# sandyresearch/chipmunk

Measured on AMD Instinct MI355X. Metric: DiT denoise steps/sec at fixed sparsity, higher is better.
Workload: dtype bf16

## Files before the change

### chipmunk_amd/csrc/attn64.hip

```cpp
#include "common.h"
#include "attn64_regs.h"
#include "attn_params.h"
#include "attn64_util.h"
#include <type_traits>

namespace {

constexpr int HD = 128;
constexpr int KT = 64;
constexpr int WROWS = 64, WGROWS = 256;
constexpr int TB = KT * HD * 2;
constexpr int NSL = 4;
constexpr int VRING = NSL * TB;
constexpr int LDS_BYTES = 2 * NSL * TB;
constexpr int PSTAGE = 64 * 128;
constexpr int LDS_BYTES_CSUM = LDS_BYTES + 4 * PSTAGE;
constexpr int CS_EXCH_BYTES = 2 * 4 * 64 * 4;
constexpr float SCALE_LOG2E = 0.08838834764f * 1.44269504089f;
constexpr float MAX_LAG = 4.0f;
#ifndef A64_ABL
#define A64_ABL 0
#endif
#ifndef A64_EB
#define A64_EB 20
#endif
#ifndef A64_EA
#define A64_EA 35
#endif
#ifndef A64_CSUM_VALU
#define A64_CSUM_VALU 1
#endif
#ifndef A64_VSPREAD
#define A64_VSPREAD 0
#endif
#ifndef A64_DMA_POS
#define A64_DMA_POS 2
#endif

constexpr int a64_ecum(int k) {
    return k <= 0 ? 0 : k <= 20 ? (k * A64_EB) / 20 : k <= 52 ? A64_EB + ((k - 20) * A64_EA) / 32
                                                              : (A64_EB + A64_EA + (k - 52) < 64 ? A64_EB + A64_EA + (k - 52) : 64);
}
constexpr int a64_cstep(int j) {
    int k = 0;
    while (a64_ecum(k) < 2 * j + 2) ++k;
    return k;
}
constexpr int a64_rk(int u) { return u == 0 ? 36 : u == 1 ? 38 : u == 2 ? 68 : 70; }
constexpr int a64_mk(int u) { return u == 0 ? 46 : u == 1 ? 48 : u == 2 ? 78 : 80; }

#ifdef ATTN64_PROF
__device__ unsigned long long g_a64_prof[4 * 8];
#define P64_DECL unsigned long long pt_ = 0, pacc_[7] = {0, 0, 0, 0, 0, 0, 0}; const bool prof_on_ = blockIdx.x == (gridDim.x / 2)
#define P64_START() do { if (prof_on_) pt_ = __builtin_amdgcn_s_memtime(); } while (0)
#define P64_MARK(i) do { if (prof_on_) { const unsigned long long n_ = __builtin_amdgcn_s_memtime(); pacc_[i] += n_ - pt_; pt_ = n_; } } while (0)
#define P64_END(w, n) do { if (prof_on_ && lane == 0) { for (int i_ = 0; i_ < 7; ++i_) g_a64_prof[(w) * 8 + i_] = pacc_[i_]; g_a64_prof[(w) * 8 + 7] = (n); } } while (0)
#else
#define P64_DECL
#define P64_START()
#define P64_MARK(i)
#define P64_END(w, n)
#endif

template <int KB, int QB, int KS>
__device__ __forceinline__ void mfma_qk(f32x16 &s) {
    constexpr int ka = 192 + (KB * 8 + KS) * 4, qa = 128 + (QB * 8 + KS) * 4;
    if constexpr (A64_ABL & 64) {
        constexpr int oa = (KB * 2 + QB) * 16;
        asm volatile("v_mfma_f32_32x32x16_bf16 a[%c0:%c1], a[%c2:%c3], a[%c4:%c5], a[%c0:%c1]" ::"i"(oa), "i"(oa + 15), "i"(ka), "i"(ka + 3), "i"(qa), "i"(qa + 3));
        return;
    }
    if constexpr (KS == 0)
        asm volatile("v_mfma_f32_32x32x16_bf16 %0, a[%c1:%c2], a[%c3:%c4], 0" : "=v"(s) : "i"(ka), "i"(ka + 3), "i"(qa), "i"(qa + 3));
    else
        asm volatile("v_mfma_f32_32x32x16_bf16 %0, a[%c1:%c2], a[%c3:%c4], %0" : "+v"(s) : "i"(ka), "i"(ka + 3), "i"(qa), "i"(qa + 3));
}
template <int QB, int DB>
__device__ __forceinline__ void mfma_pv(const u32x4 &vf, const u32x4 &pf) {
    constexpr int oa = (QB * 4 + DB) * 16;
    asm volatile("v_mfma_f32_32x32x16_bf16 a[%c2:%c3], %0, %1, a[%c2:%c3]" ::"v"(vf), "v"(pf), "i"(oa), "i"(oa + 15));
}
template <int KB, int KS, int SLOT>
__device__ __forceinline__ void lds_k(uint32_t addr) {
    constexpr int ka = 192 + (KB * 8 + KS) * 4;
    asm volatile("ds_read_b128 a[%c1:%c2], %0 offset:%c3" ::"v"(addr), "i"(ka), "i"(ka + 3), "i"(SLOT * TB + KB * 8192) : "memory");
}
__device__ __forceinline__ void cs_pair16x2(float &a, float &b, float &c, float &d) {
    asm volatile("v_permlane16_swap_b32 %0, %1\n\tv_permlane16_swap_b32 %2, %3\n\tv_add_f32 %0, %0, %1\n\tv_add_f32 %2, %2, %3"
                 : "+v"(a), "+v"(b), "+v"(c), "+v"(d));
}
__device__ __forceinline__ void cs_pair8(float &a, const float &b) {
    asm volatile("v_add_f32_dpp %0, %0, %0 row_mirror row_mask:0xf bank_mask:0x3\n\t"
                 "v_add_f32_dpp %0, %1, %1 row_mirror row_mask:0xf bank_mask:0xc" : "+v"(a) : "v"(b));
}
__device__ __forceinline__ void cs_pair4(float &a, const float &b) {
    asm volatile("v_add_f32_dpp %0, %0, %0 row_half_mirror row_mask:0xf bank_mask:0x5\n\t"
                 "v_add_f32_dpp %0, %1, %1 row_half_mirror row_mask:0xf bank_mask:0xa" : "+v"(a) : "v"(b));
}
template <int CTRL>
__device__ __forceinline__ float cs_pair_quad(float a, float b, bool hi) {
    const float keep = hi ? b : a, give = hi ? a : b;
    return keep + __uint_as_float((uint32_t)__builtin_amdgcn_update_dpp(0, (int)__float_as_uint(give), CTRL, 0xf, 0xf, true));
}
__global__ __launch_bounds__(256) void knorm_max_kernel(const uint16_t *k, const int64_t ks0, const int64_t ks1, const int64_t ks2, int H, int Nk,
                                                        float *out) {
    const int bh = blockIdx.y, b = bh / H, h = bh - b * H;
    const uint16_t *kb = k + b * ks0 + h * ks1;
    const int grp = threadIdx.x >> 4, li = threadIdx.x & 15;
    float best = 0.f;
#pragma unroll 4
    for (int row = blockIdx.x * 16 + grp; row < Nk; row += gridDim.x * 16) {
        const u32x4 v = *(const u32x4 *)(kb + (int64_t)row * ks2 + li * 8);
        float ss = 0.f;
#pragma unroll
        for (int e = 0; e < 4; ++e) {
            const float lo = __uint_as_float(v[e] << 16), hi = __uint_as_float(v[e] & 0xffff0000u);
            ss = __builtin_fmaf(lo, lo, ss);
            ss = __builtin_fmaf(hi, hi, ss);
        }
        best = fmaxf(best, row16_sum(ss));
    }
    __shared__ float red[256];
    red[threadIdx.x] = best;
    __syncthreads();
    for (int st = 128; st > 0; st >>= 1) {
        if ((int)threadIdx.x < st) red[threadIdx.x] = fmaxf(red[threadIdx.x], red[threadIdx.x + st]);
        __syncthreads();
    }
    if (threadIdx.x == 0) atomicMax((unsigned int *)(out + bh), __float_as_uint(__builtin_sqrtf(red[0])));
}

template <int MODE>
__global__ __launch_bounds__(256) __attribute__((amdgpu_waves_per_eu(1, 1))) void attn64_kernel(const AttnParams p) {
    constexpr bool GATHER = MODE == 1 || MODE == 2, INPLACE = MODE == 2;
    constexpr bool CSUM = MODE == 3;
    extern __shared__ __attribute__((aligned(16))) unsigned char smem[];
    const int tid = threadIdx.x, lane = tid & 63;
    const int w = __builtin_amdgcn_readfirstlane(tid >> 6);
    const int l31 = lane & 31, hf = lane >> 5, l15 = lane & 15, lg = lane >> 4;
// ... 43 lines not shown
#pragma unroll
                for (int j = 0; j < 16; ++j) {
                    int pos = base + j;
                    pos = pos < irow.width ? pos : irow.width - 1;
                    dst[j] = idx[pos];
                }
            }
#pragma unroll
            for (int j = 0; j < 16; ++j) dst[j] = max(0, min(dst[j], p.Nk - 1));
        };
        auto all_k = [&](const int (&src)[16], int slot) {
#pragma unroll
            for (int pc = 0; pc < 16; ++pc) blds16(krsrc, __umul24((uint32_t)src[pc], kstride_b) + kswz[pc & 3], 0, smem + slot * TB + pc * 1024);
        };
        auto all_v = [&](const int (&src)[16], int slot) {
#pragma unroll
            for (int pc = 0; pc < 16; ++pc) blds16(vrsrc, __umul24((uint32_t)src[pc], vstride_b) + vswz, 0, smem + VRING + slot * TB + pc * 1024);
        };
        load_idx(0, ir[0]), load_idx(1, ir[1]), load_idx(2, ir[2]), load_idx(3, ir[3]);
        all_k(ir[0], 0);
        all_k(ir[1], 1), all_v(ir[0], 3);
        all_k(ir[2], 2), all_v(ir[0], 0);
        all_k(ir[3], 3), all_v(ir[1], 1);
        load_idx(4, ir[0]);
        asm volatile("s_waitcnt vmcnt(0)" ::: "memory");
        __syncthreads();
        auto loader_tile = [&](auto slc, int t) __attribute__((always_inline)) {
            constexpr int SL = decltype(slc)::value;
            asm volatile("s_waitcnt vmcnt(63)" ::: "memory");
            __builtin_amdgcn_s_barrier();
            load_idx(t + 5, ir[(SL + 1) & 3]);
            all_k(ir[SL], SL);
            all_v(ir[(SL + 2) & 3], (SL + 2) & 3);
        };
        for (int tb = 0;; tb += 4) {
            loader_tile(ic<0>{}, tb);
            if (tb >= T4) break;
            loader_tile(ic<1>{}, tb + 1);
            loader_tile(ic<2>{}, tb + 2);
            loader_tile(ic<3>{}, tb + 3);
        }
        asm volatile("s_waitcnt vmcnt(0)" ::: "memory");
        if (nsp > 1) {
            __syncthreads();
            __syncthreads();
            if (*(volatile int *)(smem) != nsp - 1) return;
            __syncthreads();
        }
        return;
    }

    asm volatile(A64_ZERO_O ::: A64_CLOBBER_ALL);
    float qss[2] = {0.f, 0.f};
    {
        const uint16_t *qp = p.q + b * p.qs[0] + h * p.qs[1];
        static_for<0, 16>([&](auto f) {
            constexpr int F = decltype(f)::value, qb = F >> 3, ks = F & 7;
            const int qrow = row0 + qb * 32 + l31;
            u32x4 val = {0u, 0u, 0u, 0u};
            if (qrow < p.Nq) val = *(const u32x4 *)(qp + (int64_t)qrow * p.qs[2] + ks * 16 + hf * 8);
            acc_write4<128 + F * 4>(val);
#pragma unroll
            for (int e = 0; e < 4; ++e) {
                const float lo = __uint_as_float(val[e] << 16), hi = __uint_as_float(val[e] & 0xffff0000u);
                qss[qb] = __builtin_fmaf(lo, lo, qss[qb]);
                qss[qb] = __builtin_fmaf(hi, hi, qss[qb]);
            }
        });
    }

    const uint32_t lds0 = (uint32_t)(uintptr_t)(__attribute__((address_space(3))) unsigned char *)smem;
    uint32_t kad[8];
#pragma unroll
    for (int ks = 0; ks < 8; ++ks) kad[ks] = lds0 + l31 * 256 + (((2 * ks + hf) ^ l15) << 4);
    uint32_t vad[4];
#pragma unroll
    for (int db = 0; db < 4; ++db)
        vad[db] = lds0 + VRING + (4 * hf + (l15 >> 2)) * 256 + (((db * 4 + 2 * (lg & 1) + ((l15 & 3) >> 1)) ^ ((l15 >> 2) << 2)) << 4) +
                  (l15 & 1) * 8;
    uint32_t kofs[4];
#pragma unroll
    for (int i = 0; i < 4; ++i) kofs[i] = (uint32_t)(w * 16 + 4 * i + lg) * kstride_b + ((uint32_t)(l15 ^ (4 * i + lg)) << 4);
    const uint32_t vofs = (uint32_t)(w * 16 + lg) * vstride_b + ((uint32_t)(l15 ^ (lg << 2)) << 4);

    const int last_base = p.Nk - KT;
    auto tile_base = [&](int T) { return T * KT < last_base ? T * KT : last_base; };
    auto issue_k1 = [&](uint32_t soff, uint32_t ldsw, int slot, int i) {
        blds16(krsrc, kofs[i], soff, smem + ldsw + slot * TB + i * 1024);
    };
    auto issue_v1 = [&](uint32_t soff, uint32_t ldsw, int slot, int i) {
        blds16(vrsrc, vofs, soff + (uint32_t)(4 * i) * vstride_b, smem + ldsw + VRING + slot * TB + i * 1024);
    };
    auto issue_k = [&](int T, int slot) {
        const uint32_t soff = (uint32_t)tile_base(T) * kstride_b;
#pragma unroll
        for (int i = 0; i < 4; ++i) issue_k1(soff, w * 4096, slot, i);
    };
    auto issue_v = [&](int T, int slot) {
        const uint32_t soff = (uint32_t)tile_base(T) * vstride_b;
#pragma unroll
        for (int i = 0; i < 4; ++i) issue_v1(soff, w * 4096, slot, i);
    };

    if constexpr (!GATHER) {
        issue_k(0, 0);
        issue_k(1, 1), issue_v(0, 3);
        issue_k(2, 2), issue_v(0, 0);
        issue_k(3, 3), issue_v(1, 1);
        asm volatile("s_waitcnt vmcnt(24)" ::: "memory");
    }
    __syncthreads();
    static_for<0, 16>([&](auto i) {
        constexpr int I = decltype(i)::value;
        lds_k<(I >> 3), (I & 7), 0>(kad[I & 7]);
    });
    asm volatile("s_waitcnt lgkmcnt(0)" ::: "memory");

    f32x16 s[4];
    float px[64];
    uint32_t pw[2][4][4] = {};
    float m[2] = {-INFINITY, -INFINITY}, nmsc[2] = {0.f, 0.f};
    float mlag[2] = {-INFINITY, -INFINITY};
    float lacc[2][2] = {{0.f, 0.f}, {0.f, 0.f}};
    float alpha[2] = {1.f, 1.f};
    float wq[2] = {0.f, 0.f}, lpq[2] = {-1.0e30f, -1.0e30f}, c4[2] = {0.f, 0.f}, c5 = 0.f;
    uint32_t csoff = 0, ex_w = 0, ex_r = 0;
    int cs_extra = 0;
    float cs_own = 0.f;
    __amdgpu_buffer_rsrc_t prsrc = krsrc;
    uint32_t pst_w = 0, pst_r = 0, csoff_mx = 0;
    u32x2 csf[8] = {};
    f32x4 csacc[2] = {{0.f, 0.f, 0.f, 0.f}, {0.f, 0.f, 0.f, 0.f}};
    float csout = 0.f;
    u32x4 cs_ones = {0x3f803f80u, 0x3f803f80u, 0x3f803f80u, 0x3f803f80u};
    if constexpr (CSUM) {
        static_assert(A64_CSUM_VALU, "the matrix-pipe column-sum probe (A64_CSUM_VALU=0) fills all 160 KiB of LDS with its P stage: no room for the exchange area of the in-workgroup combine; build round 5's tree for it");
        pin(cs_ones);
        const uint32_t pst = lds0 + LDS_BYTES + (uint32_t)w * PSTAGE;
        pst_w = pst + l31 * 128 + ((uint32_t)(hf ^ (l31 & 7)) << 4);
        const int prow = lg * 4 + (l15 >> 2);
        pst_r = pst + prow * 128 + ((uint32_t)(((l15 & 3) >> 1) ^ (prow & 7)) << 4) + (l15 & 1) * 8;
        csoff_mx = 2u * (uint32_t)(16 * lg + 8 * ((l15 >> 2) & 1) + 4 * (l15 >> 3) + (l15 & 3));
#pragma unroll
        for (int qb = 0; qb < 2; ++qb) {
            const int qrow = row0 + qb * 32 + l31;
            const float pl = qrow < p.Nq ? p.p_in[(int64_t)bh * p.Nq + qrow] : 0.f;
            lpq[qb] = pl > 0.f ? __builtin_amdgcn_logf(pl) : -1.0e30f;
        }
        const int rr = ((lane >> 4) & 1) | (((lane >> 3) & 1) << 1) | (((lane >> 2) & 1) << 2);
        csoff = 2u * (uint32_t)(32 * (lane & 1) + (rr & 3) + 8 * (2 * ((lane >> 1) & 1) + (rr >> 2)) + 4 * hf);
        const int nA = 3 - (4 * g) % 3;
        const int lead = w < nA ? 0 : nA, members = w < nA ? nA : 4 - nA;
        cs_extra = w == lead ? members : 0;
        ex_w = lds0 + LDS_BYTES + (uint32_t)w * 256u + (uint32_t)lane * 4u;
        ex_r = lds0 + LDS_BYTES + (uint32_t)(lead + 1) * 256u + (uint32_t)lane * 4u;
        prsrc = make_rsrc(p.cs_part + ((int64_t)bh * (p.G * 2) + (g * 2 + (w < nA ? 0 : 1))) * p.cs_pstride);
    }
#pragma unroll
    for (int e = 0; e < 64; ++e) px[e] = e < 20 ? 0.f : -INFINITY;

    auto vfrag_read = [&](auto dbc, auto offc) __attribute__((always_inline)) {
        constexpr int DB = decltype(dbc)::value, OFF = decltype(offc)::value;
        u32x2 lo, hi;
        asm volatile("ds_read_b64_tr_b16 %0, %2 offset:%c3\n\tds_read_b64_tr_b16 %1, %2 offset:%c4"
                     : "=&v"(lo), "=&v"(hi) : "v"(vad[DB]), "i"(OFF), "i"(OFF + 2048) : "memory");
        return (u32x4){lo[0], lo[1], hi[0], hi[1]};
    };

    static_assert(64 - A64_EB - A64_EA >= 0 && 64 - A64_EB - A64_EA <= 9, "the last steps must finish before gap 12 of the next PV phase");
    auto ecum = [](int k) constexpr { return a64_ecum(k); };
    auto finish_step = [&](auto kk, auto uwc) __attribute__((always_inline)) {
        constexpr int K = decltype(kk)::value;
        constexpr bool UW = decltype(uwc)::value != 0;
        if constexpr (!(A64_ABL & 1)) {
            static_for<ecum(K), ecum(K + 1)>([&](auto ii) {
                constexpr int I = decltype(ii)::value;
                if constexpr (A64_ABL & 32) px[I] = px[I] * 0.5f;
                else px[I] = __builtin_amdgcn_exp2f(px[I]);
                pin(px[I]);
            });
            static_for<ecum(K - 1), ecum(K)>([&](auto ii) {
                constexpr int I = decltype(ii)::value;
                lacc[(I >> 3) & 1][I & 1] += px[I];
                pin(lacc[(I >> 3) & 1][I & 1]);
            });
            static_for<(ecum(K - 1) >> 1), (ecum(K) >> 1)>([&](auto jj) {
                constexpr int J = decltype(jj)::value, I = 2 * J;
                pw[(I >> 3) & 1][I >> 4][(I & 7) >> 1] = pack_bf16x2(px[I], px[I + 1]);
                pin(pw[(I >> 3) & 1][I >> 4][(I & 7) >> 1]);
            });
            if constexpr (CSUM && UW && !A64_CSUM_VALU) {
                static_assert(a64_cstep(8 * 1 + 7) + 1 < a64_rk(0) && a64_cstep(8 * 3 + 7) + 1 < a64_rk(2), "a unit is read after its second fragment is stored");
                static_for<0, 4>([&](auto uu) {
                    constexpr int U = decltype(uu)::value, S = (U & 1) * 4;
                    if constexpr (K == a64_mk(U) || K == a64_mk(U) + 1) {
                        constexpr int H2 = K - a64_mk(U);
                        if constexpr (H2 == 0 && (U & 1) == 0)
                            asm volatile("s_waitcnt lgkmcnt(0)" : "+v"(csf[0]), "+v"(csf[1]), "+v"(csf[2]), "+v"(csf[3]), "+v"(csf[4]), "+v"(csf[5]), "+v"(csf[6]), "+v"(csf[7]) :: "memory");
                        const u32x4 fr = {csf[S + 2 * H2][0], csf[S + 2 * H2][1], csf[S + 2 * H2 + 1][0], csf[S + 2 * H2 + 1][1]};
                        if constexpr (H2 == 0) asm volatile("v_mfma_f32_16x16x32_bf16 %0, %1, %2, 0" : "=&v"(csacc[U & 1]) : "v"(cs_ones), "v"(fr));
                        else asm volatile("v_mfma_f32_16x16x32_bf16 %0, %1, %2, %0" : "+v"(csacc[U & 1]) : "v"(cs_ones), "v"(fr));
                    }
                    if constexpr (K == a64_mk(U) + 3) {
                        if constexpr (U == 0) csout = csacc[0][0];
                        else csout = lg == U ? csacc[U & 1][0] : csout;
                        pin(csout);
                    }
                    if constexpr (K == a64_rk(U) || K == a64_rk(U) + 1) {
                        constexpr int H2 = K - a64_rk(U);
                        uint32_t ad = pst_r;
                        if constexpr (U != 0) ad ^= (uint32_t)(U << 5);
                        asm volatile("ds_read_b64_tr_b16 %0, %2 offset:%c3\n\tds_read_b64_tr_b16 %1, %2 offset:%c4"
                                     : "=&v"(csf[S + 2 * H2]), "=&v"(csf[S + 2 * H2 + 1]) : "v"(ad), "i"(H2 * 4096), "i"(H2 * 4096 + 2048) : "memory");
                    }
                });
                static_for<0, 8>([&](auto ii) {
                    constexpr int U = decltype(ii)::value >> 1, QW = decltype(ii)::value & 1;
                    if constexpr (K == a64_cstep(8 * U + 4 * QW + 3) + 1) {
                        uint32_t ad = pst_w;
                        if constexpr (U != 0) ad ^= (uint32_t)(U << 5);
                        const u32x4 pf = {pw[QW][U][0], pw[QW][U][1], pw[QW][U][2], pw[QW][U][3]};
                        asm volatile("ds_write_b128 %0, %1 offset:%c2" ::"v"(ad), "v"(pf), "i"(QW * 4096) : "memory");
                    }
                });
            } else if constexpr (CSUM) {
                static_for<ecum(K - 3), ecum(K - 2)>([&](auto ii) {
                    constexpr int I = decltype(ii)::value;
                    if constexpr (UW) {
                        if constexpr (((I >> 3) & 1) == 1) { px[I] += px[I - 8]; pin(px[I]); }
                    } else {
                        if constexpr (((I >> 3) & 1) == 0) px[I] *= wq[0];
                        else px[I] = __builtin_fmaf(px[I], wq[1], px[I - 8]);
                        pin(px[I]);
                    }
                });
                static_for<ecum(K - 4), ecum(K - 3)>([&](auto ii) {
                    constexpr int I = decltype(ii)::value;
                    if constexpr ((I & 11) == 11) cs_pair16x2(px[I - 3], px[I - 2], px[I - 1], px[I]);
                });
                static_for<ecum(K - 5), ecum(K - 4)>([&](auto ii) {
                    constexpr int I = decltype(ii)::value;
                    if constexpr ((I & 11) == 11) cs_pair8(px[I - 3], px[I - 1]);
                });
                static_for<ecum(K - 6), ecum(K - 5)>([&](auto ii) {
                    constexpr int I = decltype(ii)::value;
                    if constexpr ((I & 15) == 15) cs_pair4(px[I - 7], px[I - 3]);
                });
                static_for<ecum(K - 7), ecum(K - 6)>([&](auto ii) {
                    constexpr int I = decltype(ii)::value;
                    if constexpr ((I & 31) == 31) { c4[I >> 5] = cs_pair_quad<0x4E>(px[I - 23], px[I - 7], (lane & 2) != 0); pin(c4[I >> 5]); }
                });
                static_for<ecum(K - 8), ecum(K - 7)>([&](auto ii) {
                    constexpr int I = decltype(ii)::value;
                    if constexpr (I == 63) { c5 = cs_pair_quad<0xB1>(c4[0], c4[1], (lane & 1) != 0); pin(c5); }
                });
            }
        }
    };

    P64_DECL;
    P64_START();
    auto tile = [&](auto slc, auto nmc, int t) __attribute__((always_inline)) {
        constexpr int SL = decltype(slc)::value;
        constexpr bool NOMAX = decltype(nmc)::value != 0;
        constexpr auto uwc = ic<(CSUM && decltype(nmc)::value == 2) ? 1 : 0>{};
        constexpr int VSL = (SL + 3) & 3;
        constexpr int KNSL = (SL + 1) & 3;
        uint32_t ldsw = w * 4096, ksoff = 0, vsoff = 0;
        if constexpr (!(A64_ABL & 16)) {
            if constexpr (!(A64_ABL & 256) && !GATHER) asm volatile("s_waitcnt vmcnt(16)" ::: "memory");
            if constexpr (!(A64_ABL & 128)) __builtin_amdgcn_s_barrier();
            if constexpr (!GATHER) {
                asm volatile("" : "+s"(ldsw));
                ksoff = (uint32_t)tile_base(t + 4) * kstride_b;
                vsoff = (uint32_t)tile_base(t + 2) * vstride_b;
            }
        }
        __builtin_amdgcn_sched_barrier(0);
        P64_MARK(0);

        u32x4 vf[16];
        static_for<0, 32>([&](auto gg) {
            constexpr int G = decltype(gg)::value;
            constexpr int ks = G >> 2, kb = (G >> 1) & 1, qb = G & 1;
            mfma_qk<kb, qb, ks>(s[kb * 2 + qb]);
            if constexpr (!(A64_ABL & 16) && !GATHER && ((A64_DMA_POS == 0 && G < 8) || (A64_DMA_POS == 2 && G >= 16 && (G & 1) == 0))) {
                constexpr int PC = A64_DMA_POS == 0 ? G : (G - 16) >> 1;
                if constexpr (PC < 4) issue_k1(ksoff, ldsw, SL, PC);
                else issue_v1(vsoff, ldsw, (SL + 2) & 3, PC - 4);
            }
            finish_step(ic<20 + G>{}, uwc);
            if constexpr (A64_VSPREAD ? (G & 1) == 0 : G < 16) {
                constexpr int f = A64_VSPREAD ? G >> 1 : G;
                if constexpr (A64_ABL & 4) vf[f] = (u32x4){(uint32_t)t, 1u, 2u, 3u};
                else vf[f] = vfrag_read(ic<(f & 3)>{}, ic<VSL * TB + (f >> 2) * 4096>{});
            }
            __builtin_amdgcn_sched_barrier(0);
        });
        P64_MARK(1);
        asm volatile("s_waitcnt lgkmcnt(0)"
                     : "+v"(vf[0]), "+v"(vf[1]), "+v"(vf[2]), "+v"(vf[3]), "+v"(vf[4]), "+v"(vf[5]), "+v"(vf[6]), "+v"(vf[7]), "+v"(vf[8]),
                       "+v"(vf[9]), "+v"(vf[10]), "+v"(vf[11]), "+v"(vf[12]), "+v"(vf[13]), "+v"(vf[14]), "+v"(vf[15]));
        __builtin_amdgcn_sched_barrier(0);
        P64_MARK(2);

        float mx[2];
        bool moved = false;
        const int dead = GATHER ? 0 : (t * KT - tile_base(t) < KT ? t * KT - tile_base(t) : KT);
        const int vleft = !GATHER ? KT : (t < ntiles ? valid - (tbeg + t) * KT : 0);
        auto phase_b_gap = [&](auto gg) __attribute__((always_inline)) {
            constexpr int G = decltype(gg)::value;
            constexpr int up = G >> 3, db = (G >> 1) & 3, qb = G & 1;
            const u32x4 pf = {pw[qb][up][0], pw[qb][up][1], pw[qb][up][2], pw[qb][up][3]};
            mfma_pv<qb, db>(vf[G >> 1], pf);
            constexpr bool UWT = decltype(uwc)::value != 0 && !A64_CSUM_VALU;
            if constexpr (G < (CSUM ? (UWT ? 32 : 17) : 12)) finish_step(ic<52 + G>{}, uwc);
            if constexpr (CSUM && G == (UWT ? 31 : 17)) {
                const uint32_t par2 = (uint32_t)(t & 1) * 1024u;
                const float mine = UWT ? csout : c5;
                if (!cs_extra) {
                    asm volatile("ds_write_b32 %0, %1" ::"v"(ex_w + (par2 ^ 1024u)), "v"(mine) : "memory");
                } else {
                    float x1 = 0.f, x2 = 0.f;
                    if (cs_extra >= 2) asm volatile("ds_read_b32 %0, %1" : "=v"(x1) : "v"(ex_r + par2) : "memory");
                    if (cs_extra >= 3) asm volatile("ds_read_b32 %0, %1 offset:256" : "=v"(x2) : "v"(ex_r + par2) : "memory");
                    asm volatile("ds_write_b32 %0, %1" ::"v"(ex_w + (par2 ^ 1024u)), "v"(mine) : "memory");
                    asm volatile("s_waitcnt lgkmcnt(1)" : "+v"(x1), "+v"(x2)::"memory");
                    const int tb2 = tile_base(t - 2), dd = (t - 2) * KT - tb2;
                    if (t > 1 && dd < KT) {
                        const uint32_t off = UWT ? csoff_mx : csoff;
                        if (dd <= 0 || (int)(off >> 1) >= dd) {
                            const uint16_t val = (uint16_t)(pack_bf16x2((cs_own + x1) + x2, 0.f) & 0xffffu);
                            if (p.probe & 16) __builtin_amdgcn_raw_buffer_store_b16(val, prsrc, off, (uint32_t)tb2 * 2u, 2);
                            else __builtin_amdgcn_raw_buffer_store_b16(val, prsrc, off, (uint32_t)tb2 * 2u, 0);
                        }
                    }
                }
                cs_own = mine;
            }
            if constexpr (!(A64_ABL & 16) && !GATHER && A64_DMA_POS == 1 && G >= 16 && (G & 1) == 0) {
                constexpr int PC = (G - 16) >> 1;
                if constexpr (PC < 4) issue_k1(ksoff, ldsw, SL, PC);
                else issue_v1(vsoff, ldsw, (SL + 2) & 3, PC - 4);
            }
            if constexpr (G < 16 && !(A64_ABL & 8)) {
                constexpr int J = G;
                lds_k<(J >> 3), (J & 7), KNSL>(kad[J & 7]);
            }
            if constexpr (G == 1 && !(A64_ABL & 2)) {
                if (!GATHER && __builtin_expect(dead > 0, 0)) {
                    int thr = dead - 4 * hf;
                    asm volatile("" : "+v"(thr));
#pragma unroll
                    for (int blk = 0; blk < 4; ++blk)
#pragma unroll
                        for (int r = 0; r < 16; ++r)
                            if ((blk >> 1) * 32 + (r & 3) + 8 * (r >> 2) < thr) s[blk][r] = -INFINITY;
                }
                if (GATHER && __builtin_expect(vleft < KT, 0)) {
                    int thr = vleft - hf;
                    asm volatile("" : "+v"(thr));
#pragma unroll
                    for (int blk = 0; blk < 4; ++blk)
#pragma unroll
                        for (int r = 0; r < 16; ++r)
                            if ((r & 3) * 16 + (blk >> 1) * 8 + 2 * (r >> 2) >= thr) s[blk][r] = -INFINITY;
                }
            }
            if constexpr (G >= 2 && G <= 9 && !(A64_ABL & 2) && !NOMAX) {
                constexpr int j = G - 2;
                constexpr int kb2 = j >> 2, r0 = (j & 3) * 4;
                if constexpr (j == 0)
                    asm volatile("v_max_f32 %0, %2, %3\n\tv_max_f32 %1, %6, %7\n\tv_max3_f32 %0, %0, %4, %5\n\tv_max3_f32 %1, %1, %8, %9"
                                 : "=&v"(mx[0]), "=&v"(mx[1])
                                 : "v"(s[0][0]), "v"(s[0][1]), "v"(s[0][2]), "v"(s[0][3]), "v"(s[1][0]), "v"(s[1][1]), "v"(s[1][2]), "v"(s[1][3]));
                else
                asm volatile("v_max3_f32 %0, %0, %2, %3\n\tv_max3_f32 %1, %1, %6, %7\n\tv_max3_f32 %0, %0, %4, %5\n\tv_max3_f32 %1, %1, %8, %9"
                             : "+v"(mx[0]), "+v"(mx[1])
                             : "v"(s[kb2 * 2][r0]), "v"(s[kb2 * 2][r0 + 1]), "v"(s[kb2 * 2][r0 + 2]), "v"(s[kb2 * 2][r0 + 3]),
                               "v"(s[kb2 * 2 + 1][r0]), "v"(s[kb2 * 2 + 1][r0 + 1]), "v"(s[kb2 * 2 + 1][r0 + 2]), "v"(s[kb2 * 2 + 1][r0 + 3]));
            }
            if constexpr (G == 10 && !(A64_ABL & 2) && !NOMAX) {
#pragma unroll
                for (int q2 = 0; q2 < 2; ++q2) {
                    float a = mx[q2], c = mx[q2];
                    lane_swap32(a, c);
                    mx[q2] = max2(a, c);
                    pin(mx[q2]);
                }
            }
            if constexpr (G >= 12 && G < 28 && !(A64_ABL & 2)) {
                static_for<(G - 12) * 4, (G - 11) * 4>([&](auto ii) {
                    constexpr int I = decltype(ii)::value;
                    constexpr int blk = (I >> 5) * 2 + ((I >> 3) & 1), r = ((I >> 4) & 1) * 8 + (I & 7);
                    px[I] = __builtin_fmaf(s[blk][r], SCALE_LOG2E, nmsc[(I >> 3) & 1]);
                    pin(px[I]);
                });
            }
            if constexpr (G >= 12) finish_step(ic<G - 12>{}, uwc);
            __builtin_amdgcn_sched_barrier(0);
        };
        static_for<0, 12>(phase_b_gap);
        P64_MARK(3);
        if constexpr (!(A64_ABL & 2) && !NOMAX) {
            constexpr float LAG_RAW = MAX_LAG / SCALE_LOG2E;
            if (__builtin_amdgcn_ballot_w64(mx[0] > mlag[0]) | __builtin_amdgcn_ballot_w64(mx[1] > mlag[1])) {
                moved = true;
#pragma unroll
                for (int q2 = 0; q2 < 2; ++q2) {
                    const float m_new = max2(m[q2], mx[q2]);
                    alpha[q2] = __builtin_amdgcn_exp2f((m[q2] - m_new) * SCALE_LOG2E);
                    lacc[q2][0] *= alpha[q2];
                    lacc[q2][1] *= alpha[q2];
                    m[q2] = m_new;
                    nmsc[q2] = -m_new * SCALE_LOG2E;
                    mlag[q2] = m_new + LAG_RAW;
                    if constexpr (CSUM) wq[q2] = fminf(__builtin_amdgcn_exp2f(m_new * SCALE_LOG2E + lpq[q2]), 1.0e37f);
                }
            }
        }
        __builtin_amdgcn_sched_barrier(0);
        P64_MARK(4);
        static_for<12, 32>(phase_b_gap);
        P64_MARK(5);
        if (__builtin_expect(moved, 0)) {
            float tmp;
            asm volatile("s_nop 7\n\ts_nop 7\n\ts_nop 7\n\t" A64_SCALE_QB0 : "=&v"(tmp) : "v"(alpha[0]));
            asm volatile(A64_SCALE_QB1 : "=&v"(tmp) : "v"(alpha[1]));
        }
        asm volatile("s_waitcnt lgkmcnt(0)" ::: "memory");
        __builtin_amdgcn_sched_barrier(0);
        P64_MARK(6);
    };

    bool nomax = false;
    if constexpr (!GATHER) {
        if (p.kmax) {
            const float km = p.kmax[bh];
            bool ok = true;
#pragma unroll
            for (int qb = 0; qb < 2; ++qb) {
                float a = qss[qb], c2 = qss[qb];
                lane_swap32(a, c2);
                const float mq = __builtin_sqrtf(a + c2) * km;
                ok = ok && (2.0f * mq * SCALE_LOG2E <= 64.0f);
                qss[qb] = mq;
            }
            nomax = __builtin_amdgcn_ballot_w64(!ok) == 0;
            if (nomax) {
#pragma unroll
                for (int qb = 0; qb < 2; ++qb) {
                    m[qb] = qss[qb], nmsc[qb] = -qss[qb] * SCALE_LOG2E, mlag[qb] = INFINITY;
                    if constexpr (CSUM) wq[qb] = fminf(__builtin_amdgcn_exp2f(qss[qb] * SCALE_LOG2E + lpq[qb]), 1.0e37f);
                }
            }
        }
    }
    bool unitw = false;
    if constexpr (CSUM) {
        if (nomax && !(p.probe & 4)) {
            bool ok = true;
#pragma unroll
            for (int qb = 0; qb < 2; ++qb) ok = ok && lpq[qb] > -1.0e29f && qss[qb] * SCALE_LOG2E + __builtin_fabsf(lpq[qb]) <= 80.0f;
            unitw = __builtin_amdgcn_ballot_w64(!ok) == 0;
            if (unitw) {
#pragma unroll
                for (int qb = 0; qb < 2; ++qb) m[qb] = -lpq[qb] / SCALE_LOG2E, nmsc[qb] = lpq[qb];
            }
        }
    }
    if (CSUM && unitw) {
        if constexpr (CSUM) {
            for (int tb = 0;; tb += 4) {
                tile(ic<0>{}, ic<2>{}, tb);
                if (tb >= T4) break;
                tile(ic<1>{}, ic<2>{}, tb + 1);
                tile(ic<2>{}, ic<2>{}, tb + 2);
                tile(ic<3>{}, ic<2>{}, tb + 3);
            }
        }
    } else if (nomax) {
        for (int tb = 0;; tb += 4) {
            tile(ic<0>{}, ic<1>{}, tb);
            if (tb >= T4) break;
            tile(ic<1>{}, ic<1>{}, tb + 1);
            tile(ic<2>{}, ic<1>{}, tb + 2);
            tile(ic<3>{}, ic<1>{}, tb + 3);
        }
    } else {
        for (int tb = 0;; tb += 4) {
            tile(ic<0>{}, ic<0>{}, tb);
            if (tb >= T4) break;
            tile(ic<1>{}, ic<0>{}, tb + 1);
            tile(ic<2>{}, ic<0>{}, tb + 2);
            tile(ic<3>{}, ic<0>{}, tb + 3);
        }
    }
    asm volatile("s_waitcnt vmcnt(0)" ::: "memory");
    P64_END(w, T4 + 1);
    if constexpr (CSUM) {
        asm volatile("s_waitcnt lgkmcnt(0)" ::: "memory");
        __builtin_amdgcn_s_barrier();
        if (cs_extra) {
            float x1 = 0.f, x2 = 0.f;
            const uint32_t par = (uint32_t)((T4 - 1) & 1) * 1024u;
            if (cs_extra >= 2) asm volatile("ds_read_b32 %0, %1" : "=v"(x1) : "v"(ex_r + par) : "memory");
            if (cs_extra >= 3) asm volatile("ds_read_b32 %0, %1 offset:256" : "=v"(x2) : "v"(ex_r + par) : "memory");
            asm volatile("s_waitcnt lgkmcnt(0)" : "+v"(x1), "+v"(x2)::"memory");
            const int tb1 = tile_base(T4 - 1), dd = (T4 - 1) * KT - tb1;
            const uint32_t off = (unitw && !A64_CSUM_VALU) ? csoff_mx : csoff;
            if (dd < KT && (dd <= 0 || (int)(off >> 1) >= dd))
                __builtin_amdgcn_raw_buffer_store_b16((uint16_t)(pack_bf16x2((cs_own + x1) + x2, 0.f) & 0xffffu), prsrc, off, (uint32_t)tb1 * 2u, 0);
        }
    }

    asm volatile("s_nop 7\n\ts_nop 7\n\ts_nop 7" ::: "memory");
    float o[128];
    static_for<0, 32>([&](auto ii) {
        constexpr int I = decltype(ii)::value;
        const f32x4 o4 = acc_read4<I * 4>();
        o[I * 4 + 0] = o4[0], o[I * 4 + 1] = o4[1], o[I * 4 + 2] = o4[2], o[I * 4 + 3] = o4[3];
    });
    float lq[2];
#pragma unroll
    for (int qb = 0; qb < 2; ++qb) {
        float lp = lacc[qb][0] + lacc[qb][1], lo2 = lp;
        lane_swap32(lp, lo2);
        lq[qb] = lp + lo2;
    }

    if constexpr (GATHER) {
        if (nsp > 1) {
            constexpr int SLICE_FLOATS = 26 * 256 * 4;
            int *ticket_s = (int *)smem;
            float *mine = p.ws + (int64_t)(slot0 + sp) * SLICE_FLOATS + tid;
#pragma unroll
            for (int i = 0; i < 128; ++i) mine[i * 192] = o[i];
            mine[128 * 192] = m[0], mine[129 * 192] = m[1], mine[130 * 192] = lq[0], mine[131 * 192] = lq[1];
            __syncthreads();
            if (tid == 0) {
                __builtin_amdgcn_fence(__ATOMIC_RELEASE, "agent");
                asm volatile("s_waitcnt vmcnt(0)" ::: "memory");
                *ticket_s = __hip_atomic_fetch_add(p.tickets + tix, 1, __ATOMIC_RELAXED, __HIP_MEMORY_SCOPE_AGENT);
            }
            __syncthreads();
            if (*ticket_s != nsp - 1) return;
            if (tid == 0) {
                __hip_atomic_store(p.tickets + tix, 0, __ATOMIC_RELAXED, __HIP_MEMORY_SCOPE_AGENT);
                __builtin_amdgcn_fence(__ATOMIC_ACQUIRE, "agent");
            }
            __syncthreads();
#pragma unroll
            for (int i = 0; i < 128; ++i) o[i] = 0.f;
            m[0] = m[1] = -INFINITY, lq[0] = lq[1] = 0.f;
            for (int s2 = 0; s2 < nsp; ++s2) {
                const float *oth = p.ws + (int64_t)(slot0 + s2) * SLICE_FLOATS + tid;
#pragma unroll
                for (int qb = 0; qb < 2; ++qb) {
                    const float ms = oth[(128 + qb) * 192], ls = oth[(130 + qb) * 192];
                    const float m_new = fmaxf(m[qb], ms);
                    if (m_new == -INFINITY) continue;
                    const float a = __builtin_amdgcn_exp2f((m[qb] - m_new) * SCALE_LOG2E);
                    const float c = __builtin_amdgcn_exp2f((ms - m_new) * SCALE_LOG2E);
                    m[qb] = m_new;
                    lq[qb] = lq[qb] * a + ls * c;
#pragma unroll
                    for (int i = 0; i < 64; ++i) o[qb * 64 + i] = o[qb * 64 + i] * a + oth[(qb * 64 + i) * 192] * c;
                }
            }
        }
    }

#pragma unroll
    for (int qb = 0; qb < 2; ++qb) {
        const float l = lq[qb];
        const float inv = l > 0.f ? __builtin_amdgcn_rcpf(l) : 0.f;
        const int qrow = row0 + qb * 32 + l31;
        if (qrow >= p.Nq) continue;
        const int64_t ooff = b * p.os[0] + h * p.os[1] + (int64_t)qrow * p.os[2] + 4 * hf;
        uint16_t *op = p.o + ooff;
#pragma unroll
        for (int i = 0; i < 16; ++i) {
            const int db = i >> 2, r4 = i & 3;
            const float *o4 = o + (qb * 4 + db) * 16 + r4 * 4;
            float x0 = o4[0] * inv, x1 = o4[1] * inv, x2 = o4[2] * inv, x3 = o4[3] * inv;
            u32x2 out;
            if constexpr (INPLACE) {
                const u32x2 old = *(const u32x2 *)(p.o_in + ooff + db * 32 + r4 * 8);
                const float a0 = round_bf16(x0 * p.o_scale), a1 = round_bf16(x1 * p.o_scale);
                const float a2 = round_bf16(x2 * p.o_scale), a3 = round_bf16(x3 * p.o_scale);
// ... 176 lines not shown
}
#endif

const float *chipmunk_knorm_max(const uint16_t *k, const int64_t ks[3], int B, int H, int Nk, hipStream_t stream) {
    if (chipmunk_get_option("attn_nomax") == 2 || (size_t)B * H * sizeof(float) > (32 << 10)) return nullptr;
    unsigned char *sc = (unsigned char *)chipmunk_scratch(stream, 64 << 10);
    if (!sc) return nullptr;
    float *km = (float *)(sc + (32 << 10));
    if (hipMemsetAsync(km, 0, (size_t)B * H * sizeof(float), stream) != hipSuccess) return nullptr;
    hipLaunchKernelGGL(knorm_max_kernel, dim3(Nk >= 4096 ? 64 : 8, B * H), dim3(256), 0, stream, k, ks[0], ks[1], ks[2], H, Nk, km);
    return km;
}

int chipmunk_dense64_launch(const void *q, const void *k, const void *v, void *o, float *l, const int64_t qs[3],
                            const int64_t ks[3], const int64_t vs[3], const int64_t os[3], int B, int H, int Nq, int Nk,
                            hipStream_t stream) {
    AttnParams p = {};
    p.q = (const uint16_t *)q, p.k = (const uint16_t *)k, p.v = (const uint16_t *)v, p.o = (uint16_t *)o;
    for (int i = 0; i < 3; ++i) p.qs[i] = qs[i], p.ks[i] = ks[i], p.vs[i] = vs[i], p.os[i] = os[i];
    p.l_out = l;
    p.B = B, p.H = H, p.Nq = Nq, p.Nk = Nk, p.G = (Nq + WGROWS - 1) / WGROWS;
    p.o_scale = 1.f;
    p.kmax = chipmunk_knorm_max(p.k, ks, B, H, Nk, stream);
    return launch64<0>(p, (int64_t)B * H * p.G, stream);
}

namespace {
__global__ __launch_bounds__(256) void cs_combine_kernel(const uint16_t *part, int pstride, uint16_t *cs, int NRB, int G, int Nq, int Nk, int cs_stride) {
    const int g = blockIdx.y, bh = blockIdx.z;
    int r0, r1;
    const int nrows = colsum_part_rows(g, NRB / 2, r0, r1);
    const uint16_t *src = part + ((int64_t)bh * NRB + r0) * pstride;
    const int64_t row1 = (int64_t)(r1 - r0) * pstride;
    uint16_t *dst = cs + ((int64_t)bh * G + g) * cs_stride;
    if (((Nk | cs_stride) & 3) == 0) {
        const int j = (blockIdx.x * 256 + threadIdx.x) * 4;
        if (j >= Nk) return;
        float acc[4];
        {
            const u32x2 x = *(const u32x2 *)(src + j);
            acc[0] = __uint_as_float(x[0] << 16), acc[1] = __uint_as_float(x[0] & 0xffff0000u);
            acc[2] = __uint_as_float(x[1] << 16), acc[3] = __uint_as_float(x[1] & 0xffff0000u);
        }
        if (nrows == 2) {
            const u32x2 x = *(const u32x2 *)(src + row1 + j);
            acc[0] += __uint_as_float(x[0] << 16), acc[1] += __uint_as_float(x[0] & 0xffff0000u);
            acc[2] += __uint_as_float(x[1] << 16), acc[3] += __uint_as_float(x[1] & 0xffff0000u);
        }
        *(u32x2 *)(dst + j) = (u32x2){pack_bf16x2(acc[0], acc[1]), pack_bf16x2(acc[2], acc[3])};
    } else {
        for (int e = 0; e < 4; ++e) {
            const int j = (blockIdx.x * 256 + threadIdx.x) * 4 + e;
            if (j >= Nk) return;
            float acc = bf16_bits_to_f32(src[j]);
            if (nrows == 2) acc += bf16_bits_to_f32(src[row1 + j]);
            dst[j] = f32_to_bf16_bits(acc);
        }
    }
}
}

int chipmunk_colsum64_launch(const AttnParams &p, hipStream_t stream) {
    static uint64_t lds_set = 0;
    ensure_dynamic_lds((const void *)colsum64_kernel, NSL * TB, lds_set);
    const int64_t grid = (int64_t)p.B * p.H * ((p.G + 3) / 4);
    hipLaunchKernelGGL(colsum64_kernel, dim3((unsigned)grid), dim3(256), NSL * TB, stream, p);
    CM_LAUNCH_CHECK();
    return CHIPMUNK_OK;
}

int chipmunk_colsum_part_stride(int Nk) { return (chipmunk_get_option("attn_cs_probe") & 1) ? Nk : (Nk + 63) & ~63; }

size_t chipmunk_colsum_part_bytes(int B, int H, int Nq, int Nk) {
    return (size_t)B * H * (((Nq + WGROWS - 1) / WGROWS) * 2) * (size_t)chipmunk_colsum_part_stride(Nk) * sizeof(uint16_t);
}

int chipmunk_dense64_colsum_launch(const AttnParams &p0, uint16_t *part, hipStream_t stream) {
    AttnParams p = p0;
    const int G192 = p.G;
    p.G = (p.Nq + WGROWS - 1) / WGROWS;
    p.cs_part = part, p.cs_pstride = chipmunk_colsum_part_stride(p.Nk);
    if (chipmunk_get_option("attn_cs_probe") & 2) p.probe |= 16;
    if (chipmunk_get_option("attn_fused_colsum") == 3) p.probe |= 4;
    p.kmax = chipmunk_knorm_max(p.k, p.ks, p.B, p.H, p.Nk, stream);
    if (int rc = launch64<3>(p, (int64_t)p.B * p.H * p.G, stream)) return rc;
    if (!p.cs) return CHIPMUNK_OK;
    hipLaunchKernelGGL(cs_combine_kernel, dim3((unsigned)((p.Nk + 1023) / 1024), (unsigned)G192, (unsigned)(p.B * p.H)), dim3(256), 0, stream,
                       part, p.cs_pstride, p.cs, p.G * 2, G192, p.Nq, p.Nk, p.cs_stride);
    CM_LAUNCH_CHECK();
    return CHIPMUNK_OK;
}

int chipmunk_csp64_launch(const AttnParams &p, int inplace, int grid, hipStream_t stream) {
    CM_CHECK(p.plan && p.tickets && p.ws, "csp64: work plan missing");
    return inplace ? launch64<2>(p, grid, stream) : launch64<1>(p, grid, stream);
}
```

Measured before the change: 0.5853.

## Rebalance V-tile DMA between waves and restructure column-sum exchange in MODE 3

In the fused column-sum attention kernel (MODE 3), the lead waves now give some V-tile load pieces to the member waves. This is meant to even out the per-wave work imbalance caused by the column-sum combine that the leads perform, and the vmcnt waits are adjusted to match each wave's role. The cross-wave column-sum exchange now uses fixed slots and double the exchange area. Its LDS read is split from its wait across gaps 17 and 21, and the exp-step schedule gets separate EB/EA constants for the CSUM path. The change adds role-specialised code paths and more LDS for the exchange, and wrong waitcnt accounting could cause races.

New measurement: 0.5850 (median of 2 runs). About the same (-0.1%).

```diff
diff --git a/chipmunk_amd/csrc/attn64.hip b/chipmunk_amd/csrc/attn64.hip
--- a/chipmunk_amd/csrc/attn64.hip
+++ b/chipmunk_amd/csrc/attn64.hip
@@ -15,7 +15,7 @@
 constexpr int LDS_BYTES = 2 * NSL * TB;
 constexpr int PSTAGE = 64 * 128;
 constexpr int LDS_BYTES_CSUM = LDS_BYTES + 4 * PSTAGE;
-constexpr int CS_EXCH_BYTES = 2 * 4 * 64 * 4;
+constexpr int CS_EXCH_BYTES = 2 * 8 * 64 * 4;
 constexpr float SCALE_LOG2E = 0.08838834764f * 1.44269504089f;
 constexpr float MAX_LAG = 4.0f;
 #ifndef A64_ABL
@@ -27,34 +27,42 @@
 #ifndef A64_EA
 #define A64_EA 35
 #endif
+#ifndef A64_EB3
+#define A64_EB3 18
+#endif
+#ifndef A64_EA3
+#define A64_EA3 39
+#endif
 #ifndef A64_CSUM_VALU
 #define A64_CSUM_VALU 1
 #endif
 #ifndef A64_VSPREAD
 #define A64_VSPREAD 0
 #endif
+#ifndef A64_GIVE
+#define A64_GIVE 2
+#endif
 #ifndef A64_DMA_POS
 #define A64_DMA_POS 2
 #endif
 
-constexpr int a64_ecum(int k) {
-    return k <= 0 ? 0 : k <= 20 ? (k * A64_EB) / 20 : k <= 52 ? A64_EB + ((k - 20) * A64_EA) / 32
-                                                              : (A64_EB + A64_EA + (k - 52) < 64 ? A64_EB + A64_EA + (k - 52) : 64);
-}
-constexpr int a64_cstep(int j) {
+constexpr int a64_ecum(int k, int EB, int EA) {
+    return k <= 0 ? 0 : k <= 20 ? (k * EB) / 20 : k <= 52 ? EB + ((k - 20) * EA) / 32 : (EB + EA + (k - 52) < 64 ? EB + EA + (k - 52) : 64);
+}
+constexpr int a64_cstep(int j, int EB, int EA) {
     int k = 0;
-    while (a64_ecum(k) < 2 * j + 2) ++k;
+    while (a64_ecum(k, EB, EA) < 2 * j + 2) ++k;
     return k;
 }
 constexpr int a64_rk(int u) { return u == 0 ? 36 : u == 1 ? 38 : u == 2 ? 68 : 70; }
 constexpr int a64_mk(int u) { return u == 0 ? 46 : u == 1 ? 48 : u == 2 ? 78 : 80; }
 
 #ifdef ATTN64_PROF
-__device__ unsigned long long g_a64_prof[4 * 8];
-#define P64_DECL unsigned long long pt_ = 0, pacc_[7] = {0, 0, 0, 0, 0, 0, 0}; const bool prof_on_ = blockIdx.x == (gridDim.x / 2)
+__device__ unsigned long long g_a64_prof[3 * 4 * 8];
+#define P64_DECL unsigned long long pt_ = 0, pacc_[7] = {0, 0, 0, 0, 0, 0, 0}; const unsigned pwg_ = blockIdx.x - gridDim.x / 2; const bool prof_on_ = pwg_ < 3u
 #define P64_START() do { if (prof_on_) pt_ = __builtin_amdgcn_s_memtime(); } while (0)
 #define P64_MARK(i) do { if (prof_on_) { const unsigned long long n_ = __builtin_amdgcn_s_memtime(); pacc_[i] += n_ - pt_; pt_ = n_; } } while (0)
-#define P64_END(w, n) do { if (prof_on_ && lane == 0) { for (int i_ = 0; i_ < 7; ++i_) g_a64_prof[(w) * 8 + i_] = pacc_[i_]; g_a64_prof[(w) * 8 + 7] = (n); } } while (0)
+#define P64_END(w, n) do { if (prof_on_ && lane == 0) { for (int i_ = 0; i_ < 7; ++i_) g_a64_prof[(pwg_ * 4 + (w)) * 8 + i_] = pacc_[i_]; g_a64_prof[(pwg_ * 4 + (w)) * 8 + 7] = (n); } } while (0)
 #else
 #define P64_DECL
 #define P64_START()
@@ -264,6 +272,16 @@
 #pragma unroll
     for (int i = 0; i < 4; ++i) kofs[i] = (uint32_t)(w * 16 + 4 * i + lg) * kstride_b + ((uint32_t)(l15 ^ (4 * i + lg)) << 4);
     const uint32_t vofs = (uint32_t)(w * 16 + lg) * vstride_b + ((uint32_t)(l15 ^ (lg << 2)) << 4);
+    int role = 0, wp = w;
+    if constexpr (MODE == 3) {
+        const int nA = 3 - (4 * g) % 3;
+        if (!(p.probe & 64)) {
+            role = (w == 0 || w == nA) ? 1 : 2;
+            if (role == 2) wp = (w - 1 - (w > nA ? 1 : 0)) == 0 ? 0 : nA;
+        }
+    }
+    const uint32_t vofs_p = (uint32_t)(wp * 16 + lg) * vstride_b + ((uint32_t)(l15 ^ (lg << 2)) << 4);
+    const int v_own = role == 1 ? 4 - A64_GIVE : 4, v_take = role == 2 ? A64_GIVE : 0;
 
     const int last_base = p.Nk - KT;
     auto tile_base = [&](int T) { return T * KT < last_base ? T * KT : last_base; };
@@ -273,6 +291,9 @@
     auto issue_v1 = [&](uint32_t soff, uint32_t ldsw, int slot, int i) {
         blds16(vrsrc, vofs, soff + (uint32_t)(4 * i) * vstride_b, smem + ldsw + VRING + slot * TB + i * 1024);
     };
+    auto issue_vp = [&](uint32_t soff, uint32_t ldswp, int slot, int i) {
+        blds16(vrsrc, vofs_p, soff + (uint32_t)(4 * i) * vstride_b, smem + ldswp + VRING + slot * TB + i * 1024);
+    };
     auto issue_k = [&](int T, int slot) {
         const uint32_t soff = (uint32_t)tile_base(T) * kstride_b;
 #pragma unroll
@@ -280,16 +301,27 @@
     };
     auto issue_v = [&](int T, int slot) {
         const uint32_t soff = (uint32_t)tile_base(T) * vstride_b;
-#pragma unroll
-        for (int i = 0; i < 4; ++i) issue_v1(soff, w * 4096, slot, i);
-    };
-
+        if constexpr (MODE == 3) {
+#pragma unroll
+            for (int i = 0; i < 4; ++i)
+                if (i < v_own) issue_v1(soff, w * 4096, slot, i);
+#pragma unroll
+            for (int i = 0; i < 4; ++i)
+                if (i >= 4 - v_take) issue_vp(soff, wp * 4096, slot, i);
+        } else {
+#pragma unroll
+            for (int i = 0; i < 4; ++i) issue_v1(soff, w * 4096, slot, i);
+        }
+    };
+
+    if constexpr (MODE == 3) *(u32x4 *)(smem + LDS_BYTES + tid * 16) = (u32x4){0u, 0u, 0u, 0u};
     if constexpr (!GATHER) {
         issue_k(0, 0);
         issue_k(1, 1), issue_v(0, 3);
         issue_k(2, 2), issue_v(0, 0);
         issue_k(3, 3), issue_v(1, 1);
-        asm volatile("s_waitcnt vmcnt(24)" ::: "memory");
+        if constexpr (MODE == 3) asm volatile("s_waitcnt vmcnt(%c0)" ::"i"(3 * (8 - A64_GIVE)) : "memory");
+        else asm volatile("s_waitcnt vmcnt(24)" ::: "memory");
     }
     __syncthreads();
     static_for<0, 16>([&](auto i) {
@@ -309,6 +341,7 @@
     uint32_t csoff = 0, ex_w = 0, ex_r = 0;
     int cs_extra = 0;
     float cs_own = 0.f;
+    float cs_x1 = 0.f, cs_x2 = 0.f;
     __amdgpu_buffer_rsrc_t prsrc = krsrc;
     uint32_t pst_w = 0, pst_r = 0, csoff_mx = 0;
     u32x2 csf[8] = {};
@@ -334,12 +367,14 @@
         const int nA = 3 - (4 * g) % 3;
         const int lead = w < nA ? 0 : nA, members = w < nA ? nA : 4 - nA;
         cs_extra = w == lead ? members : 0;
-        ex_w = lds0 + LDS_BYTES + (uint32_t)w * 256u + (uint32_t)lane * 4u;
-        ex_r = lds0 + LDS_BYTES + (uint32_t)(lead + 1) * 256u + (uint32_t)lane * 4u;
+        const int st4 = w < nA ? 0 : 4;
+        ex_w = lds0 + LDS_BYTES + (uint32_t)(st4 + (w == lead ? 2 : w - lead - 1)) * 256u + (uint32_t)lane * 4u;
+        ex_r = w == lead ? lds0 + LDS_BYTES + (uint32_t)st4 * 256u + (uint32_t)lane * 4u : ex_w;
         prsrc = make_rsrc(p.cs_part + ((int64_t)bh * (p.G * 2) + (g * 2 + (w < nA ? 0 : 1))) * p.cs_pstride);
     }
-#pragma unroll
-    for (int e = 0; e < 64; ++e) px[e] = e < 20 ? 0.f : -INFINITY;
+    constexpr int EB = CSUM ? A64_EB3 : A64_EB, EA = CSUM ? A64_EA3 : A64_EA;
+#pragma unroll
+    for (int e = 0; e < 64; ++e) px[e] = e < EB ? 0.f : -INFINITY;
 
     auto vfrag_read = [&](auto dbc, auto offc) __attribute__((always_inline)) {
         constexpr int DB = decltype(dbc)::value, OFF = decltype(offc)::value;
@@ -349,8 +384,8 @@
         return (u32x4){lo[0], lo[1], hi[0], hi[1]};
     };
 
-    static_assert(64 - A64_EB - A64_EA >= 0 && 64 - A64_EB - A64_EA <= 9, "the last steps must finish before gap 12 of the next PV phase");
-    auto ecum = [](int k) constexpr { return a64_ecum(k); };
+    static_assert(64 - EB - EA >= 0 && 64 - EB - EA <= 9, "the last steps must finish before gap 12 of the next PV phase");
+    auto ecum = [](int k) constexpr { return a64_ecum(k, EB, EA); };
     auto finish_step = [&](auto kk, auto uwc) __attribute__((always_inline)) {
         constexpr int K = decltype(kk)::value;
         constexpr bool UW = decltype(uwc)::value != 0;
@@ -372,7 +407,7 @@
                 pin(pw[(I >> 3) & 1][I >> 4][(I & 7) >> 1]);
             });
             if constexpr (CSUM && UW && !A64_CSUM_VALU) {
-                static_assert(a64_cstep(8 * 1 + 7) + 1 < a64_rk(0) && a64_cstep(8 * 3 + 7) + 1 < a64_rk(2), "a unit is read after its second fragment is stored");
+                static_assert(a64_cstep(8 * 1 + 7, EB, EA) + 1 < a64_rk(0) && a64_cstep(8 * 3 + 7, EB, EA) + 1 < a64_rk(2), "a unit is read after its second fragment is stored");
                 static_for<0, 4>([&](auto uu) {
                     constexpr int U = decltype(uu)::value, S = (U & 1) * 4;
                     if constexpr (K == a64_mk(U) || K == a64_mk(U) + 1) {
@@ -398,7 +433,7 @@
                 });
                 static_for<0, 8>([&](auto ii) {
                     constexpr int U = decltype(ii)::value >> 1, QW = decltype(ii)::value & 1;
-                    if constexpr (K == a64_cstep(8 * U + 4 * QW + 3) + 1) {
+                    if constexpr (K == a64_cstep(8 * U + 4 * QW + 3, EB, EA) + 1) {
                         uint32_t ad = pst_w;
                         if constexpr (U != 0) ad ^= (uint32_t)(U << 5);
                         const u32x4 pf = {pw[QW][U][0], pw[QW][U][1], pw[QW][U][2], pw[QW][U][3]};
@@ -442,18 +477,23 @@
 
     P64_DECL;
     P64_START();
-    auto tile = [&](auto slc, auto nmc, int t) __attribute__((always_inline)) {
+    auto tile = [&](auto slc, auto nmc, auto rolec, int t) __attribute__((always_inline)) {
         constexpr int SL = decltype(slc)::value;
+        constexpr int ROLE = decltype(rolec)::value;
+        static_assert(ROLE == 0 || (CSUM && A64_DMA_POS == 2 && A64_GIVE >= 1 && A64_GIVE <= 2), "the uneven split is MODE 3's, pieces in phase A gaps 16..31");
+        constexpr int NPC = ROLE == 1 ? 8 - A64_GIVE : ROLE == 2 ? 8 + A64_GIVE : 8;
         constexpr bool NOMAX = decltype(nmc)::value != 0;
         constexpr auto uwc = ic<(CSUM && decltype(nmc)::value == 2) ? 1 : 0>{};
         constexpr int VSL = (SL + 3) & 3;
         constexpr int KNSL = (SL + 1) & 3;
-        uint32_t ldsw = w * 4096, ksoff = 0, vsoff = 0;
+        uint32_t ldsw = w * 4096, ldswp = wp * 4096, ksoff = 0, vsoff = 0;
         if constexpr (!(A64_ABL & 16)) {
-            if constexpr (!(A64_ABL & 256) && !GATHER) asm volatile("s_waitcnt vmcnt(16)" ::: "memory");
+            if constexpr (!(A64_ABL & 256) && !GATHER && ROLE == 0) asm volatile("s_waitcnt vmcnt(16)" ::: "memory");
+            if constexpr (!(A64_ABL & 256) && !GATHER && ROLE != 0) asm volatile("s_waitcnt vmcnt(%c0)" ::"i"(2 * NPC) : "memory");
             if constexpr (!(A64_ABL & 128)) __builtin_amdgcn_s_barrier();
             if constexpr (!GATHER) {
                 asm volatile("" : "+s"(ldsw));
+                if constexpr (ROLE == 2) asm volatile("" : "+s"(ldswp));
                 ksoff = (uint32_t)tile_base(t + 4) * kstride_b;
                 vsoff = (uint32_t)tile_base(t + 2) * vstride_b;
             }
@@ -469,8 +509,10 @@
             if constexpr (!(A64_ABL & 16) && !GATHER && ((A64_DMA_POS == 0 && G < 8) || (A64_DMA_POS == 2 && G >= 16 && (G & 1) == 0))) {
                 constexpr int PC = A64_DMA_POS == 0 ? G : (G - 16) >> 1;
                 if constexpr (PC < 4) issue_k1(ksoff, ldsw, SL, PC);
-                else issue_v1(vsoff, ldsw, (SL + 2) & 3, PC - 4);
-            }
+                else if constexpr (!(ROLE == 1 && PC - 4 >= 4 - A64_GIVE)) issue_v1(vsoff, ldsw, (SL + 2) & 3, PC - 4);
+            }
+            if constexpr (ROLE == 2 && !(A64_ABL & 16) && G >= 32 - 2 * A64_GIVE && (G & 1) == 1)
+                issue_vp(vsoff, ldswp, (SL + 2) & 3, 4 - A64_GIVE + ((G - (33 - 2 * A64_GIVE)) >> 1));
             finish_step(ic<20 + G>{}, uwc);
             if constexpr (A64_VSPREAD ? (G & 1) == 0 : G < 16) {
                 constexpr int f = A64_VSPREAD ? G >> 1 : G;
@@ -497,17 +539,19 @@
             mfma_pv<qb, db>(vf[G >> 1], pf);
             constexpr bool UWT = decltype(uwc)::value != 0 && !A64_CSUM_VALU;
             if constexpr (G < (CSUM ? (UWT ? 32 : 17) : 12)) finish_step(ic<52 + G>{}, uwc);
-            if constexpr (CSUM && G == (UWT ? 31 : 17)) {
-                const uint32_t par2 = (uint32_t)(t & 1) * 1024u;
+            constexpr int CS_XG = 17;
+            static_assert(!UWT, "the matrix-pipe probe has its sums in gap 31 only: see the static_assert on A64_CSUM_VALU");
+            if constexpr (CSUM && G == CS_XG) {
+                const uint32_t par2 = (uint32_t)(t & 1) * 2048u;
+                asm volatile("ds_read_b32 %0, %1" : "=v"(cs_x1) : "v"(ex_r + par2) : "memory");
+                asm volatile("ds_read_b32 %0, %1 offset:256" : "=v"(cs_x2) : "v"(ex_r + par2) : "memory");
+                asm volatile("ds_write_b32 %0, %1" ::"v"(ex_w + (par2 ^ 2048u)), "v"(UWT ? csout : c5) : "memory");
+            }
+            if constexpr (CSUM && G == CS_XG + 4) {
                 const float mine = UWT ? csout : c5;
-                if (!cs_extra) {
-                    asm volatile("ds_write_b32 %0, %1" ::"v"(ex_w + (par2 ^ 1024u)), "v"(mine) : "memory");
-                } else {
-                    float x1 = 0.f, x2 = 0.f;
-                    if (cs_extra >= 2) asm volatile("ds_read_b32 %0, %1" : "=v"(x1) : "v"(ex_r + par2) : "memory");
-                    if (cs_extra >= 3) asm volatile("ds_read_b32 %0, %1 offset:256" : "=v"(x2) : "v"(ex_r + par2) : "memory");
-                    asm volatile("ds_write_b32 %0, %1" ::"v"(ex_w + (par2 ^ 1024u)), "v"(mine) : "memory");
-                    asm volatile("s_waitcnt lgkmcnt(1)" : "+v"(x1), "+v"(x2)::"memory");
+                asm volatile("s_waitcnt lgkmcnt(1)" : "+v"(cs_x1), "+v"(cs_x2)::"memory");
+                if (cs_extra) {
+                    const float x1 = cs_x1, x2 = cs_x2;
                     const int tb2 = tile_base(t - 2), dd = (t - 2) * KT - tb2;
                     if (t > 1 && dd < KT) {
                         const uint32_t off = UWT ? csoff_mx : csoff;
@@ -651,31 +695,39 @@
             }
         }
     }
-    if (CSUM && unitw) {
-        if constexpr (CSUM) {
-            for (int tb = 0;; tb += 4) {
-                tile(ic<0>{}, ic<2>{}, tb);
-                if (tb >= T4) break;
-                tile(ic<1>{}, ic<2>{}, tb + 1);
-                tile(ic<2>{}, ic<2>{}, tb + 2);
-                tile(ic<3>{}, ic<2>{}, tb + 3);
-            }
-        }
+    auto run = [&](auto nmc, auto rolec) __attribute__((always_inline)) {
+        for (int tb = 0;; tb += 4) {
+            tile(ic<0>{}, nmc, rolec, tb);
+            if (tb >= T4) break;
+            tile(ic<1>{}, nmc, rolec, tb + 1);
+            tile(ic<2>{}, nmc, rolec, tb + 2);
+            tile(ic<3>{}, nmc, rolec, tb + 3);
+        }
+    };
+    auto run_role = [&](auto nmc) __attribute__((always_inline)) {
+        if (role == 1) run(nmc, ic<1>{});
+        else if (role == 2) run(nmc, ic<2>{});
+        else run(nmc, ic<0>{});
+    };
+    if constexpr (CSUM) {
+        if (unitw) run_role(ic<2>{});
+        else if (nomax) run_role(ic<1>{});
+        else run_role(ic<0>{});
     } else if (nomax) {
         for (int tb = 0;; tb += 4) {
-            tile(ic<0>{}, ic<1>{}, tb);
+            tile(ic<0>{}, ic<1>{}, ic<0>{}, tb);
             if (tb >= T4) break;
-            tile(ic<1>{}, ic<1>{}, tb + 1);
-            tile(ic<2>{}, ic<1>{}, tb + 2);
-            tile(ic<3>{}, ic<1>{}, tb + 3);
+            tile(ic<1>{}, ic<1>{}, ic<0>{}, tb + 1);
+            tile(ic<2>{}, ic<1>{}, ic<0>{}, tb + 2);
+            tile(ic<3>{}, ic<1>{}, ic<0>{}, tb + 3);
         }
     } else {
         for (int tb = 0;; tb += 4) {
-            tile(ic<0>{}, ic<0>{}, tb);
+            tile(ic<0>{}, ic<0>{}, ic<0>{}, tb);
             if (tb >= T4) break;
-            tile(ic<1>{}, ic<0>{}, tb + 1);
-            tile(ic<2>{}, ic<0>{}, tb + 2);
-            tile(ic<3>{}, ic<0>{}, tb + 3);
+            tile(ic<1>{}, ic<0>{}, ic<0>{}, tb + 1);
+            tile(ic<2>{}, ic<0>{}, ic<0>{}, tb + 2);
+            tile(ic<3>{}, ic<0>{}, ic<0>{}, tb + 3);
         }
     }
     asm volatile("s_waitcnt vmcnt(0)" ::: "memory");
@@ -685,9 +737,9 @@
         __builtin_amdgcn_s_barrier();
         if (cs_extra) {
             float x1 = 0.f, x2 = 0.f;
-            const uint32_t par = (uint32_t)((T4 - 1) & 1) * 1024u;
-            if (cs_extra >= 2) asm volatile("ds_read_b32 %0, %1" : "=v"(x1) : "v"(ex_r + par) : "memory");
-            if (cs_extra >= 3) asm volatile("ds_read_b32 %0, %1 offset:256" : "=v"(x2) : "v"(ex_r + par) : "memory");
+            const uint32_t par = (uint32_t)((T4 - 1) & 1) * 2048u;
+            asm volatile("ds_read_b32 %0, %1" : "=v"(x1) : "v"(ex_r + par) : "memory");
+            asm volatile("ds_read_b32 %0, %1 offset:256" : "=v"(x2) : "v"(ex_r + par) : "memory");
             asm volatile("s_waitcnt lgkmcnt(0)" : "+v"(x1), "+v"(x2)::"memory");
             const int tb1 = tile_base(T4 - 1), dd = (T4 - 1) * KT - tb1;
             const uint32_t off = (unitw && !A64_CSUM_VALU) ? csoff_mx : csoff;
@@ -1030,6 +1082,7 @@
     p.cs_part = part, p.cs_pstride = chipmunk_colsum_part_stride(p.Nk);
     if (chipmunk_get_option("attn_cs_probe") & 2) p.probe |= 16;
     if (chipmunk_get_option("attn_fused_colsum") == 3) p.probe |= 4;
+    p.probe |= chipmunk_get_option("attn_variant") & (4 | 64);
     p.kmax = chipmunk_knorm_max(p.k, p.ks, p.B, p.H, p.Nk, stream);
     if (int rc = launch64<3>(p, (int64_t)p.B * p.H * p.G, stream)) return rc;
     if (!p.cs) return CHIPMUNK_OK;
```
